# YuemingJin/STswinCL

Measured on AMD Instinct MI355X. Metric: input frames/s, TswinPlus fwd+bwd+Adam, 4-frame 512x512 clips, higher is better.
Workload: dtype bf16; 1 GPU; BASELINE.json configs[1]: TswinPlus(12) seg train step, 4 clips/GPU x T=4 frames x 3x512x512, swin res (64,64), OHEM-CE, Adam; T=4 because the reference asserts it (swin_512.py:313); clips_per_gpu=4, frames_per_clip=4, parallelism=dp1, graph_requested=True

## Files before the change

### include/stswin_hip.h

```cpp
#ifndef STSWIN_HIP_H
#define STSWIN_HIP_H
#ifdef __cplusplus
extern "C" {
#endif

#define STSWIN_GF_GELU 1
#define STSWIN_GF_RESID 2
#define STSWIN_GF_MUL_DGELU 4
#define STSWIN_GF_OUT_F32 8
#define STSWIN_GF_ACCUM 16
#define STSWIN_GF_RELU 32
#define STSWIN_GF_MUL_R 8192
#define STSWIN_GF_C2_DGELU 16384
#define STSWIN_GF_CS_PARTIAL 32768
#define STSWIN_GF_CS_SQ 65536
#define STSWIN_GF_TAPSKIP (1 << 29)
#define STSWIN_GF_BIG 128
#define STSWIN_GF_MID 512
#define STSWIN_GF_NOPIPE 1024
#define STSWIN_GF_HALF 2048
#define STSWIN_GF_M32PP (1u << 31)
#define STSWIN_GF_W4R (1 << 30)
#define STSWIN_GF_ROT 4096
#define STSWIN_GF_NOBIG 256
// ... 86 lines not shown
#define STSWIN_VAR_TN_RING_BSEG 23
#define STSWIN_VAR_TN_128x128 30
#define STSWIN_VAR_TN_128x128_W4 31
#define STSWIN_VAR_TN_ROWS 32
#define STSWIN_VAR_TN_SLABS_F32 0x1000
#define STSWIN_VAR_TN_SLABS_BF16 0x2000
#define STSWIN_VAR_TN_FUSED 0x8000
#define STSWIN_VAR_TN_TAPMINOR 0x4000
#define STSWIN_TN_OUT_TAPMINOR (1 << 25)
int stswin_gemm_nt_qkv_fp8(const void* A, long lda, const int* a_rows, const void* B, long ldb, void* out8, long ld8, float* scales,
                           long ld_scales, const float* bias, int M, int N, int Kseg, float scale, int scale_cols, int rows_per_problem,
                           int head_dim, void* stream);
int stswin_win_attn_fwd_f8(const void* qkv8, long ld8, const float* scales, long ld_scales, void* out, long ldo, const float* biasT,
                           const float* maskT, int nB_, int nW, int T_frames, int ws, int heads, int C, int bias_windows,
                           const int* bias_index, void* stream);
int stswin_win_attn_bwd_f8(const void* qkv8, long ld8, const float* scales, long ld_scales, const void* dout, long lddo, void* dqkv, long lddq,
                           const float* biasT, const float* maskT, float* dbiasT, float* dqkv_colsum, int nB_, int nW, int T_frames, int ws,
                           int heads, int C, float scale, int bias_windows, const int* bias_index, float* scratch, long scratch_floats,
                           void* stream);
int stswin_last_variant(int family);
int stswin_tuning_build(void);

int stswin_slab_fold(const float* ws, long slab_stride, long ws_batch_stride, int nslabs, int seg_len, int nseg, float* out0, float* out1,
                     float* out2, long out_batch_stride, int batch, int accumulate, void* stream);

int stswin_fold_defer(int on, void* stream);
int stswin_fold_flush(void* stream);

long stswin_colsum_scratch(int M, int N);
int stswin_colsum(int dtype, const void* y, long ldy, float* out, int M, int N, float* scratch, void* stream);

int stswin_layernorm_fwd(int dtype, const void* x, long ldx, const int* rows, int S, int Cseg, void* y, long ldy,
                         const float* gamma, const float* beta, float* mean, float* rstd, int M, float eps, void* stream);
int stswin_layernorm_bwd(int dtype, const void* dy, long lddy, const void* x, long ldx, const int* rows, int S, int Cseg,
                         const float* gamma, const float* mean, const float* rstd, void* dx, long lddx, float* dgamma,
                         float* dbeta, int M, int accumulate_dx,
                         float* dxsum ,
                         float* scratch ,
                         void* stream);
int stswin_layernorm_bwd_add(int dtype, const void* dy, long lddy, const void* x, long ldx, const int* rows, int S, int Cseg,
                             const float* gamma, const float* mean, const float* rstd, const void* add, long ldadd, void* dx, long lddx,
                             float* dgamma, float* dbeta, int M, float* dxsum, float* scratch, void* stream);
long stswin_layernorm_bwd_scratch(int M, int C);

int stswin_vec_gather(const float* v, const int* map, float* out, int n, float fill, void* stream);
int stswin_vec_gather_multi(int count, const float* const* v, const int* map, float* const* out, int n, const float* fill, void* stream);

int stswin_bias_expand(const float* table, const long* index, const float* mask, float* out, int N, int heads, int nW,
                       void* stream);
int stswin_bias_expand_multi(int count, const float* const* table, const long* const* index, const float* const* mask, float* const* out,
                             const int* N, const int* heads, const int* nW, void* stream);
int stswin_bias_scatter(const float* dbiasT, const int* order, const int* offs, float* dtable, int N, int heads, int table_rows, int nslabs,
                        void* stream);

int stswin_win_attn_fwd(int dtype, const void* qkv, long ld, void* out, long ldo, const float* biasT, const float* maskT,
                        int nB_, int nW, int T_frames, int ws, int heads, int C, int bias_windows,
                        const int* bias_index, void* stream);
int stswin_win_attn_qkv_fwd(const void* x, long ldx, long x_rows, const int* rmap, const void* w, long ldw, const float* bqkv, void* qkv_out,
                            long ldq, void* out, long ldo, const float* biasT, int nB_, int nW, int T_frames, int ws, int heads, int C,
                            float scale, int bias_windows, const int* bias_index, void* stream);
int stswin_win_attn_fwd_fp8(const void* qkv, long ld, void* out, long ldo, const float* biasT, const float* maskT, int nB_, int nW,
                            int T_frames, int ws, int heads, int C, int bias_windows, const int* bias_index, void* stream);
int stswin_win_attn_bwd(int dtype, const void* qkv, long ld, const void* dout, long lddo, void* dqkv, long lddq,
                        const float* biasT, const float* maskT, float* dbiasT,
                        float* dqkv_q_colsum ,
                        int nB_, int nW, int T_frames, int ws,
                        int heads, int C, float scale, int bias_windows, const int* bias_index,
                        float* scratch , long scratch_floats, void* stream);
long stswin_win_attn_bwd_scratch(int nB_, int ws, int heads, int C);

int stswin_colstats(int dtype, const void* x, long ldx, float* sum , float* sumsq , int M, int C, int groups, int unit_rows,
                    float* scratch , void* stream);
long stswin_colstats_scratch(int dtype, int M, int C, int groups, int unit_rows);
int stswin_cs_group_reduce(const float* table, int M, int N, int groups, int unit_rows, float* sum, float* sumsq, void* stream);

int stswin_bn_table_finalize(const float* table, int M, int N, int groups, int unit_rows, float* mean, float* rstd,
                             float* running_mean, float* running_var, float eps, float momentum, void* stream);
int stswin_bn_finalize(int dtype, const void* x, long ldx, const float* sum, const float* sumsq, float* mean, float* rstd,
                       float* running_mean, float* running_var, int M, int C, int groups, float eps, float momentum,
                       int unit_rows, void* stream);
int stswin_bn_apply(int dtype, const void* x, long ldx, const float* mean, const float* rstd, const float* gamma,
                    const float* beta, const void* resid, long ldr, void* y, long ldy, int M, int C, int groups, int relu,
                    int unit_rows, void* stream);
int stswin_bn_bwd(int dtype, const void* dy, long lddy, const void* x, long ldx,
                  const void* y ,
                  long ldy, const float* mean, const float* rstd, const float* gamma, const float* beta ,
                  float* s1, float* s2, void* dx, long lddx, void* dresid, long lddr,
                  int M, int C, int groups, int relu, int training,
                  int phase ,
                  long rows_total , int unit_rows,
                  float* group_sums ,
                  float* scratch ,
                  void* stream);
long stswin_bn_bwd_scratch(int dtype, int M, int C, int groups, int unit_rows);
int stswin_bn_relu_pool(int dtype, const void* x, long ldx, const float* mean, const float* rstd, const float* gamma, const float* beta,
                        void* out, long ldo, unsigned char* arg, int frames, int H, int W, int C, int groups, int unit_rows, void* stream);
int stswin_rows_broadcast(int dtype, const float* v, void* out, long ldo, int M, int C, int groups, float scale,
                          int accumulate, void* stream);
int stswin_bilinear(int dtype, const void* in, long ldi, void* out, long ldo, int frames, int h, int w, int H, int W, int C,
                    int backward, void* stream);
int stswin_logits_upsample(int dtype, const void* tokens, long ldt, void* nchw, int frames, int h, int w, int H, int W,
                           int nc, int backward, void* stream);

int stswin_ce_fwd(int dtype, const void* logits, const long* labels, float* loss, float* stats, int frames, long HW, int nc,
                  int ignore_index, float thresh, void* stream);
#define STSWIN_OHEM_WORK_BYTES (3 * 2048 * 12 + 48)
int stswin_ohem_select(const float* loss, long n, long n_min, float thresh, const float* stats, void* work, long work_bytes,
                       float* value, float* sel, void* stream);
int stswin_ce_bwd(int dtype, const void* logits, const long* labels, const float* loss, const float* sel,
                  const float* gscale, void* dlogits, int frames, long HW, int nc, int ignore_index, void* stream);

int stswin_contrast_fwd(int dtype, const void* Q, long ldq, const void* const* K5, long ldk, const int* lq,
                        const int* const* lk5, float* pos, float* all, int N, int HW, int C, void* stream);

int stswin_contrast_bank_fwd(int dtype, const void* Q, long ldq, const int* lq, int M, int C, int q_sets, int q_block,
                             const void* bank, long ldb, const int* lb, int maps, int seg, int bank_block, int groups,
                             const int* gmap , float inv_tau, float* pos, float* all,
                             float* rowmax, float* lse, float* workspace, long workspace_floats, void* stream);
int stswin_contrast_bank_fwd_unit(int dtype, const void* Q, long ldq, const int* lq, int M, int C, int q_sets, int q_block,
                             const void* bank, long ldb, const int* lb, int maps, int seg, int bank_block, int groups,
                             const int* gmap , float inv_tau, float* pos, float* all,
                             float* rowmax, float* lse, float* workspace, long workspace_floats, void* stream);
int stswin_contrast_class_sums(int dtype, const void* bank, long ldb, const int* lb, int maps, int seg, int bank_block, int C,
                               int ncls, float* ksum, float* scratch , void* stream);
long stswin_contrast_class_sums_scratch(int maps, int seg, int bank_block, int C, int ncls);
int stswin_contrast_bank_dq(const float* dpos, const float* dneg, const float* cnt, const int* lq, const float* ksum, float* dq,
                            long lddq, int M, int C, int q_sets, int q_block, int seg, int bank_block, int ncls, int groups, const int* gmap,
                            void* stream);

int stswin_rownorm_scatter(int dtype, const void* X, long ldx, void* Y, long ldy, float* inv, int R, int C, int views, int HW, int samples,
                           void* stream);
int stswin_rownorm_scatter_bwd(int dtype, const void* X, long ldx, const float* inv, const float* dY, long lddy, void* dX, long lddx, int R,
                               int C, int views, int HW, int samples, void* stream);
int stswin_labels_resize(const float* const* masks, int maps, int N, int Hs, int Ws, int h, int w, int* lb, void* stream);
int stswin_label_counts(const int* lq, const int* lb, int M, int maps, int seg, int q_sets, int q_block, int bank_block, int ncls, int groups,
                        const int* gmap, int* hist, float* cnt, void* stream);
int stswin_pair_loss(const float* pos, const float* all, const float* cnt, int M, int groups, int q_sets, int visible, float* loss,
                     void* stream);
int stswin_pair_loss_bwd(const float* pos, const float* all, const float* cnt, const float* dloss, int M, int groups, int q_sets, int visible,
                         float* dpos, float* dneg, void* stream);

int stswin_upsample_argmax(int dtype, const void* logits, unsigned char* labels, const long* gt, int* counts, int frames,
                           int nc, int h, int w, int H, int W, void* stream);
int stswin_upsample_argmax_cm(int dtype, const void* logits, unsigned char* labels, const long* gt, unsigned long long* cm, int ncm,
                              int align_corners, int frames, int nc, int h, int w, int H, int W, void* stream);

int stswin_frame_ingest(const unsigned char* in, unsigned char* tmp, float* out, int n, int Hs, int Ws, int H, int W,
                        const int* hbounds, const int* hcoef, int hksize, const int* vbounds, const int* vcoef, int vksize,
                        const float* lut, void* stream);
int stswin_frame_ingest_planes(const unsigned char* in, unsigned char* tmp, float* out, int n, int Hs, int Ws, int H, int W,
                               const int* hbounds, const int* hcoef, int hksize, const int* vbounds, const int* vcoef, int vksize,
                               const float* lut, void* stream);
int stswin_clip_assemble(int dtype, void* ring, const void* fresh, void* clips, const int* table, int B, int n_store, int slots,
                         int n_fresh, long frame_elems, void* stream);

int stswin_multi_tensor(int mode, int count, void* const* p, const void* const* g, void* const* m, void* const* v,
                        const int* n, float lr, float b1, float b2, float eps, float wd, float c1, float c2, void* stream);

int stswin_multi_tensor_lars(int count, void* const* p, const void* const* g, void* const* m, const int* n, float* norms,
                             long norms_floats, float lr, float momentum, float wd, float trust_coef, float eps, int first, int adaptive,
                             void* stream);

int stswin_optim_tick(int kind, int* counter, float* hyper, double a, double b, void* stream);
int stswin_multi_tensor_dev(int mode, int count, void* const* p, const void* const* g, void* const* m, void* const* v, const int* n,
                            const float* hyper, float b1, float b2, float eps, float wd, int first, void* stream);
int stswin_multi_tensor_lars_dev(int count, void* const* p, const void* const* g, void* const* m, const int* n, float* norms,
// ... 13 lines not shown
```

### stswincl_amd/csrc/headops.hip

```cpp
#include "common.h"
#include <cstdlib>

static int reduce_rows_per_chunk(int group_rows, int other_blocks, int nrl) {
  int rpc = 8 * nrl;
  while (rpc < 64 * nrl && (long)other_blocks * ((group_rows + 2 * rpc - 1) / (2 * rpc)) >= 1024) rpc *= 2;
  return rpc;
}
static int bn_bwd_rows(long rows_all_groups, int col_blocks, int nrl, int max_rows) {
  static const int tgt_red = getenv("STSWIN_BN_RED_WGS") ? atoi(getenv("STSWIN_BN_RED_WGS")) : 512;
  static const int tgt_dx = getenv("STSWIN_BN_DX_WGS") ? atoi(getenv("STSWIN_BN_DX_WGS")) : 2048;
  const int tgt = max_rows > 32 ? tgt_red : tgt_dx;
  int rows = 8;
  while (rows < max_rows && (long)col_blocks * (rows_all_groups / ((long)2 * rows * nrl)) >= tgt) rows *= 2;
  return rows;
}

DEVI long group_row0(int g, int ch, int rows_per_chunk, int group_rows, int unit, int G) {
  if (unit <= 0) return (long)g * group_rows;
  return ((long)((ch * rows_per_chunk) / unit) * (G - 1) + g) * unit;
}
DEVI long group_first_row(int g, int group_rows, int unit) { return unit > 0 ? (long)g * unit : (long)g * group_rows; }
static int fit_chunk(int rpc, int unit) {
  if (unit <= 0) return rpc;
  while (rpc > 1 && unit % rpc) rpc >>= 1;
// ... 473 lines not shown
    return;
  }
  float mx = -3.0e38f;
  for (int c = 0; c < nc; ++c) mx = fmaxf(mx, to_f32<TL>(b[(long)c * HW]));
  float s = 0.f;
  for (int c = 0; c < nc; ++c) s += expf(to_f32<TL>(b[(long)c * HW]) - mx);
  const float inv = 1.f / s;
  for (int c = 0; c < nc; ++c) {
    const float pr = expf(to_f32<TL>(b[(long)c * HW]) - mx) * inv;
    d[(long)c * HW] = from_f32<TL>(wgt * (pr - (c == lab ? 1.f : 0.f)));
  }
}

#define PACK_OF(dt) ((dt) == 0 ? 8 : 4)
#define DISPATCH_T(dt, CALL_BF16, CALL_F32) do { if ((dt) == 0) { CALL_BF16; } else { CALL_F32; } } while (0)

static int colstats_geometry(int dtype, int M, int C, int groups, int unit_rows, int* cpb_o, int* rpc_o, int* cpg_o) {
  if (C % PACK_OF(dtype) || groups <= 0 || M % groups) return -1401;
  if (unit_rows > 0 && M % ((long)groups * unit_rows)) return -1405;
  const int ppr = C / PACK_OF(dtype), cpb = pick_cpb(ppr);
  const int gr = M / groups, rpc = fit_chunk(reduce_rows_per_chunk(gr, groups * ((ppr + cpb - 1) / cpb), 256 / cpb), unit_rows);
  if (rpc <= 0) return -1405;
  *cpb_o = cpb; *rpc_o = rpc; *cpg_o = (gr + rpc - 1) / rpc;
  return 0;
}
extern "C" long stswin_colstats_scratch(int dtype, int M, int C, int groups, int unit_rows) {
  int cpb, rpc, cpg;
  const int rc = colstats_geometry(dtype, M, C, groups, unit_rows, &cpb, &rpc, &cpg);
  return rc ? rc : (long)groups * cpg * 2 * C;
}

extern "C" int stswin_colstats(int dtype, const void* x, long ldx, float* sum, float* sumsq, int M, int C, int groups,
                               int unit_rows, float* scratch, void* stream) {
  int cpb, rpc, cpg;
  const int rc = colstats_geometry(dtype, M, C, groups, unit_rows, &cpb, &rpc, &cpg);
  if (rc) return rc;
  if (ldx % PACK_OF(dtype)) return -1401;
  if (!scratch) return -1406;
  const int ppr = C / PACK_OF(dtype), gr = M / groups;
  dim3 grid((ppr + cpb - 1) / cpb, groups * cpg);
  hipStream_t st = (hipStream_t)stream;
  if (sumsq)
    DISPATCH_T(dtype, hipLaunchKernelGGL((colstats_kernel<bf16, true>), grid, dim3(256), 0, st, (const bf16*)x, ldx, scratch, C, gr, cpg, rpc, cpb, unit_rows),
               hipLaunchKernelGGL((colstats_kernel<float, true>), grid, dim3(256), 0, st, (const float*)x, ldx, scratch, C, gr, cpg, rpc, cpb, unit_rows));
  else
    DISPATCH_T(dtype, hipLaunchKernelGGL((colstats_kernel<bf16, false>), grid, dim3(256), 0, st, (const bf16*)x, ldx, scratch, C, gr, cpg, rpc, cpb, unit_rows),
               hipLaunchKernelGGL((colstats_kernel<float, false>), grid, dim3(256), 0, st, (const float*)x, ldx, scratch, C, gr, cpg, rpc, cpb, unit_rows));
  const int rf = stswin_fold_launch(scratch, 2L * C, (long)cpg * 2 * C, cpg, C, sumsq ? 2 : 1, sum, sumsq, nullptr, C, groups, 1, st);
  if (rf) return rf;
  STSWIN_CHECK_LAUNCH();
  return 0;
}

extern "C" int stswin_bn_finalize(int dtype, const void* x, long ldx, const float* sum, const float* sumsq, float* mean,
                                  float* rstd, float* running_mean, float* running_var, int M, int C, int groups, float eps,
                                  float momentum, int unit_rows, void* stream) {
  if (groups <= 0 || M % groups) return -1401;
  hipStream_t st = (hipStream_t)stream;
  dim3 grid((C + 255) / 256);
  DISPATCH_T(dtype, hipLaunchKernelGGL(bn_finalize_kernel<bf16>, grid, dim3(256), 0, st, (const bf16*)x, ldx, sum, sumsq, mean, rstd, running_mean, running_var, C, groups, M / groups, eps, momentum, unit_rows),
             hipLaunchKernelGGL(bn_finalize_kernel<float>, grid, dim3(256), 0, st, (const float*)x, ldx, sum, sumsq, mean, rstd, running_mean, running_var, C, groups, M / groups, eps, momentum, unit_rows));
  STSWIN_CHECK_LAUNCH();
  return 0;
}

extern "C" int stswin_bn_apply(int dtype, const void* x, long ldx, const float* mean, const float* rstd, const float* gamma,
                               const float* beta, const void* resid, long ldr, void* y, long ldy, int M, int C, int groups,
                               int relu, int unit_rows, void* stream) {
  const int pk = PACK_OF(dtype);
  if (C % pk || ldx % pk || ldy % pk || (resid && ldr % pk) || groups <= 0 || M % groups) return -1402;
  const int ppr = C / pk, cpb = pick_cpb(ppr);
  if (unit_rows > 0 && M % ((long)groups * unit_rows)) return -1405;
  const int gr = M / groups, rpc = fit_chunk(8 * (256 / cpb), unit_rows);
  if (rpc <= 0) return -1405;
  const int cpg = (gr + rpc - 1) / rpc;
  dim3 grid((ppr + cpb - 1) / cpb, groups * cpg);
  hipStream_t st = (hipStream_t)stream;
  DISPATCH_T(dtype, hipLaunchKernelGGL(bn_apply_kernel<bf16>, grid, dim3(256), 0, st, (const bf16*)x, ldx, mean, rstd, gamma, beta, (const bf16*)resid, ldr, (bf16*)y, ldy, C, gr, cpg, rpc, relu, cpb, unit_rows),
             hipLaunchKernelGGL(bn_apply_kernel<float>, grid, dim3(256), 0, st, (const float*)x, ldx, mean, rstd, gamma, beta, (const float*)resid, ldr, (float*)y, ldy, C, gr, cpg, rpc, relu, cpb, unit_rows));
  STSWIN_CHECK_LAUNCH();
  return 0;
}

static int bn_bwd_geometry(int dtype, int M, int C, int groups, int unit_rows, int* cpb_o, int* rpc_o, int* rpc2_o) {
  const int pk = PACK_OF(dtype);
  if (C % pk || groups <= 0 || M % groups) return -1403;
  if (unit_rows > 0 && M % ((long)groups * unit_rows)) return -1405;
  const int ppr = C / pk, cpb = pick_cpb(ppr), xb = (ppr + cpb - 1) / cpb, nrl = 256 / cpb;
  const int rpc = fit_chunk(bn_bwd_rows(M, xb, nrl, 64) * nrl, unit_rows);
  const int rpc2 = fit_chunk(bn_bwd_rows(M, xb, nrl, 32) * nrl, unit_rows);
  if (rpc <= 0 || rpc2 <= 0) return -1405;
  *cpb_o = cpb; *rpc_o = rpc; *rpc2_o = rpc2;
  return 0;
}
extern "C" long stswin_bn_bwd_scratch(int dtype, int M, int C, int groups, int unit_rows) {
  int cpb, rpc, rpc2;
  const int rc = bn_bwd_geometry(dtype, M, C, groups, unit_rows, &cpb, &rpc, &rpc2);
  return rc ? rc : (long)groups * ((M / groups + rpc - 1) / rpc) * 2 * C;
}

extern "C" int stswin_bn_bwd(int dtype, const void* dy, long lddy, const void* x, long ldx, const void* y, long ldy,
                             const float* mean, const float* rstd, const float* gamma, const float* beta, float* s1, float* s2,
                             void* dx, long lddx, void* dresid, long lddr, int M, int C, int groups, int relu, int training,
                             int phase, long rows_total, int unit_rows, float* gsum, float* scratch, void* stream) {
  const int pk = PACK_OF(dtype);
  int cpb, rpc, rpc2;
  const int rc = bn_bwd_geometry(dtype, M, C, groups, unit_rows, &cpb, &rpc, &rpc2);
  if (rc) return rc;
  if (ldx % pk || lddy % pk || lddx % pk || (relu && y && ldy % pk)) return -1403;
  if (relu && !y && !beta) return -1404;
  if (phase != 2 && !scratch) return -1406;
  const int ppr = C / pk, gr = M / groups;
  const int cpg = (gr + rpc - 1) / rpc;
  dim3 g1((ppr + cpb - 1) / cpb, groups * cpg);
  const int cpg2 = (gr + rpc2 - 1) / rpc2;
  dim3 g2((ppr + cpb - 1) / cpb, groups * cpg2);
  hipStream_t st = (hipStream_t)stream;
  const float inv_n = 1.0f / (float)(rows_total > 0 ? rows_total : gr);
  if (phase != 2) {
    DISPATCH_T(dtype, hipLaunchKernelGGL(bn_bwd_reduce_kernel<bf16>, g1, dim3(256), 0, st, (const bf16*)dy, lddy, (const bf16*)x, ldx, (const bf16*)y, ldy, mean, rstd, scratch, C, gr, cpg, rpc, relu, cpb, gamma, beta, unit_rows),
               hipLaunchKernelGGL(bn_bwd_reduce_kernel<float>, g1, dim3(256), 0, st, (const float*)dy, lddy, (const float*)x, ldx, (const float*)y, ldy, mean, rstd, scratch, C, gr, cpg, rpc, relu, cpb, gamma, beta, unit_rows));
    const int rf = stswin_fold_launch(scratch, 2L * C, (long)cpg * 2 * C, cpg, C, 2, s1, s2, nullptr, C, groups, 1, st);
    if (rf) return rf;
  }
  if (phase != 1)
  DISPATCH_T(dtype, hipLaunchKernelGGL(bn_bwd_dx_kernel<bf16>, g2, dim3(256), 0, st, (const bf16*)dy, lddy, (const bf16*)x, ldx, (const bf16*)y, ldy, mean, rstd, gamma, s1, s2, (bf16*)dx, lddx, (bf16*)dresid, lddr, C, gr, cpg2, rpc2, relu, training, cpb, inv_n, beta, unit_rows, gsum),
             hipLaunchKernelGGL(bn_bwd_dx_kernel<float>, g2, dim3(256), 0, st, (const float*)dy, lddy, (const float*)x, ldx, (const float*)y, ldy, mean, rstd, gamma, s1, s2, (float*)dx, lddx, (float*)dresid, lddr, C, gr, cpg2, rpc2, relu, training, cpb, inv_n, beta, unit_rows, gsum));
  STSWIN_CHECK_LAUNCH();
  return 0;
}

template <typename T>
__global__ __launch_bounds__(256) void bn_relu_pool_kernel(const T* x, long ldx, const float* mean, const float* rstd, const float* gamma,
                                                            const float* beta, T* out, long ldo, unsigned char* arg, int frames, int H,
                                                            int W, int Hp, int Wp, int C, int G, int group_rows, int unit) {
  constexpr int PACK = TT<T>::PACK;
  const int ppr = C / PACK, Hb = (Hp + 1) >> 1, Wb = (Wp + 1) >> 1;
  const long idx = (long)blockIdx.x * 256 + threadIdx.x;
  if (idx >= (long)frames * Hb * Wb * ppr) return;
  const int c = (int)(idx % ppr) * PACK;
  const long pb = idx / ppr;
  const int xb = (int)(pb % Wb), yb = (int)((pb / Wb) % Hb);
  const long f = pb / ((long)Wb * Hb);
  const long row0 = f * H * W;
  const int g = unit > 0 ? (int)((row0 / unit) % G) : (int)(row0 / group_rows);
  float sc[8], sh[8], best[4][8];
  unsigned char ba[4][8];
#pragma unroll
  for (int e = 0; e < PACK; ++e) {
    const float rs = rstd[(long)g * C + c + e] * gamma[c + e];
    sc[e] = rs;
    sh[e] = beta[c + e] - mean[(long)g * C + c + e] * rs;
#pragma unroll
    for (int o = 0; o < 4; ++o) { best[o][e] = -3.0e38f; ba[o][e] = 255; }
  }
  const int y0 = 4 * yb - 1, x0 = 4 * xb - 1;
#pragma unroll
  for (int iy = 0; iy < 5; ++iy) {
    const int yy = y0 + iy;
    if (yy < 0 || yy >= H) continue;
#pragma unroll
    for (int ix = 0; ix < 5; ++ix) {
      const int xx = x0 + ix;
      if (xx < 0 || xx >= W) continue;
      Vec16<T> v, z;
      v.v = *(const decltype(v.v)*)(x + (row0 + (long)yy * W + xx) * ldx + c);
// ... 497 lines not shown
```

### stswincl_amd/headops.py

```python
from __future__ import annotations

import os
import weakref
from typing import List, Optional, Sequence, Tuple

import torch
import torch.nn.functional as F

from . import hip
from .ops import compute_dtype, _f32

KGRAN = 64


_INDEX_MAPS = {}
_TORCH_PADVEC = os.environ.get("STSWIN_TORCH_PADVEC") == "1"
_BN_KEEP_Y = os.environ.get("STSWIN_BN_KEEP_Y") == "1"


class Layout:

    def __init__(self, segs: Sequence[Tuple[int, int, int]], width: int):
        self.segs, self.width = list(segs), width
        self.logical = sum(s[1] for s in self.segs)
# ... 362 lines not shown
def combine_bn_stats(mean_r: torch.Tensor, m2_r: torch.Tensor, n_r: torch.Tensor):
    n = n_r.sum()
    w = (n_r / n).view(-1, 1, 1)
    mean = (mean_r * w).sum(0)
    m2 = (m2_r + n_r.view(-1, 1, 1) * (mean_r - mean) ** 2).sum(0)
    return mean, m2 / n, n


def refuse_replica(module) -> None:
    if getattr(module, "_is_replica", False):
        raise hip.StswinHipError(
            "stswincl_amd modules do not run as nn.DataParallel replicas (several GPUs driven by threads of one process). Use one "
            "process per GPU instead: `python -m torch.distributed.run --nproc-per-node N train.py` with "
            "torch.nn.parallel.DistributedDataParallel or stswincl_amd.dp.GradBucketReducer (see INTEGRATION.md, 'Data parallel'); "
            "nn.DataParallel(model, device_ids=[torch.cuda.current_device()]) - a single device - is fine.")


COLLECTIVES: dict = {}


def _sync_world(bn) -> int:
    import torch.distributed as dist
    if isinstance(bn, torch.nn.SyncBatchNorm) and dist.is_available() and dist.is_initialized():
        return dist.get_world_size()
    return 1


def rowmajor(t: torch.Tensor, dt) -> torch.Tensor:
    t = t.detach()
    if t.dtype != dt:
        t = t.to(dt)
    if (t.dim() == 2 and t.stride(1) == 1 and (t.stride(0) * t.element_size()) % 16 == 0 and t.data_ptr() % 16 == 0
            and t.stride(0) >= t.shape[1]):
        return t
    return t.contiguous()


class ConcatColsFn(torch.autograd.Function):

    @staticmethod
    def forward(ctx, buf, widths, *parts):
        off = 0
        for w_, p_ in zip(widths, parts):
            assert p_.data_ptr() == buf.data_ptr() + off * buf.element_size() and p_.shape[1] == w_ and p_.stride(0) == buf.stride(0), \
                "ConcatColsFn: a part does not live in its column slice of the buffer"
            off += w_
        assert off == buf.shape[1]
        ctx.widths = widths
        return buf.view_as(buf)

    @staticmethod
    def backward(ctx, g):
        outs, off = [], 0
        for w_ in ctx.widths:
            outs.append(g[:, off:off + w_])
            off += w_
        return (None, None, *outs)


def concat_buffer(rows: int, widths, dt, device):
    buf = torch.empty(rows, sum(widths), dtype=dt, device=device)
    views, off = [], 0
    for w_ in widths:
        views.append(buf[:, off:off + w_])
        off += w_
    return buf, views


class BNTokFn(torch.autograd.Function):

    @staticmethod
    def forward(ctx, x, gamma, beta, running_mean, running_var, training, relu, resid, groups, lay, eps, momentum, world=1,
                unit=0, stats=None, link=None, out=None):
        ctx.link = link
        dt = compute_dtype(x)
        X = x.detach().to(dt)
        M, Cp = X.shape
        assert Cp == lay.width
        fused_pad = training and world == 1 and not lay.is_identity
        if fused_pad:
            gp, bp, rm_p, rv_p = lay.pad_vecs([gamma, beta, running_mean, running_var], [0.0, 0.0, 0.0, 1.0])
        else:
            gp, bp = lay.pad_vec(gamma), lay.pad_vec(beta)
        rows_total = 0
        if training and world > 1:
            import torch.distributed as dist
            n_loc = M // groups
            s, ss = hip.colstats(X, groups=groups, unit=unit)
            pivot = (X.view(-1, unit, Cp)[:groups, 0, :] if unit > 0 else X.view(groups, n_loc, Cp)[:, 0, :]).float()
            mean_l = pivot + s / n_loc
            m2_l = ss - s * s / n_loc
            pack = torch.stack([mean_l, m2_l, torch.full_like(mean_l, float(n_loc))])
            allp = torch.empty(world * 3, *pack.shape[1:], dtype=pack.dtype, device=pack.device)
            dist.all_gather_into_tensor(allp, pack)
            COLLECTIVES["syncbn_all_gather"] = COLLECTIVES.get("syncbn_all_gather", 0) + 1
            allp = allp.view(world, 3, *pack.shape[1:])
            n_r = allp[:, 2, 0, 0]
            mean, var, n_tot = combine_bn_stats(allp[:, 0], allp[:, 1], n_r)
            rstd = torch.rsqrt(var + eps)
            unbias = n_tot / (n_tot - 1).clamp(min=1)
            ctx.sum_scale = float(n_loc) / n_tot
            rm, rv = lay.pad_vec(running_mean), lay.pad_vec(running_var, 1.0)
            for g in range(groups):
                rm = (1 - momentum) * rm + momentum * mean[g]
                rv = (1 - momentum) * rv + momentum * var[g] * unbias
            running_mean.copy_(lay.unpad_vec(rm))
            running_var.copy_(lay.unpad_vec(rv))
            mean, rstd = mean.contiguous(), rstd.contiguous()
        elif training:
            raw = stats is not None and groups <= 32 and ((unit % 256 == 0) if unit > 0 else ((M // groups) % 256 == 0))

            def finalize(rm, rv):
                if raw:
                    return hip.bn_table_finalize(stats, M, rm, rv, groups, eps, momentum, unit=unit)
                s, ss = hip.colstats(X, groups=groups, unit=unit)
                return hip.bn_finalize(X, s, ss, rm, rv, groups, eps, momentum, unit=unit)

            if lay.is_identity:
                mean, rstd = finalize(running_mean, running_var)
            else:
                mean, rstd = finalize(rm_p, rv_p)
                lay.unpad_vecs([rm_p, rv_p], into=[running_mean, running_var])
        else:
            mean = lay.pad_vec(running_mean).view(1, Cp).expand(groups, Cp).contiguous()
            rstd = torch.rsqrt(lay.pad_vec(running_var, 1.0) + eps).view(1, Cp).expand(groups, Cp).contiguous()
        if out is not None:
            assert out.shape == (M, Cp) and out.dtype == dt and out.stride(1) == 1
            y = out.view_as(out)
        else:
            y = torch.empty(M, Cp, dtype=dt, device=x.device)
        R = resid.detach().to(dt) if resid is not None else None
        hip.bn_apply(X, mean, rstd, gp, bp, y, resid=R, groups=groups, relu=relu, unit=unit)
        ctx.cfg = (training, relu, groups, lay, dt, x.dtype, resid is not None, world, rows_total)
        ctx.unit = unit
        keep_y = relu and (resid is not None or _BN_KEEP_Y)
        ctx.save_for_backward(X, y if keep_y else None, mean, rstd, gp, bp if relu else None)
        return y

    @staticmethod
    def backward(ctx, dy):
        X, y, mean, rstd, gp, bp = ctx.saved_tensors
        training, relu, groups, lay, dt, in_dtype, has_res, world, rows_total = ctx.cfg
        g = rowmajor(dy, dt)
        dx = torch.empty_like(X)
        dres = torch.empty_like(X) if has_res else None
        if training and world > 1:
            import torch.distributed as dist
            s1, s2 = hip.bn_bwd(g, X, y if relu else None, mean, rstd, gp, dx, dres, groups, relu, training, phase=1, beta=bp,
                                unit=ctx.unit)
            loc1, loc2 = s1.clone(), s2.clone()
            both = torch.stack([s1, s2])
            dist.all_reduce(both)
            COLLECTIVES["syncbn_all_reduce"] = COLLECTIVES.get("syncbn_all_reduce", 0) + 1
            both = both * ctx.sum_scale
            hip.bn_bwd(g, X, y if relu else None, mean, rstd, gp, dx, dres, groups, relu, training, phase=2,
                       sums=(both[0].contiguous(), both[1].contiguous()), rows_total=0, beta=bp, unit=ctx.unit)
            s1, s2 = loc1, loc2
        else:
            gs = torch.empty(2, X.shape[1], dtype=torch.float32, device=X.device) if groups > 1 else None
            s1, s2 = hip.bn_bwd(g, X, y if relu else None, mean, rstd, gp, dx, dres, groups, relu, training, beta=bp, unit=ctx.unit,
                                group_sums=gs)
            if gs is not None:
                s1, s2, groups = gs[0:1], gs[1:2], 1
        if groups > 1:
            if s1._base is not None and s2._base is s1._base and s2.storage_offset() == s1.storage_offset() + s1.numel():
                both = torch.as_strided(s1, (2, groups, s1.shape[-1]), (groups * s1.shape[-1], s1.shape[-1], 1)).sum(1)
                s1, s2 = both[0:1], both[1:2]
            else:
                s1, s2 = s1.sum(0, keepdim=True), s2.sum(0, keepdim=True)
        if lay.is_identity:
            dgamma, dbeta = s2[0], s1[0]
        else:
            dgamma, dbeta = lay.unpad_vecs([s2[0].contiguous(), s1[0].contiguous()])
        dres = dres.to(in_dtype) if has_res else None
        if dres is not None and ctx.link is not None:
            ctx.link.put(dres)
            dres = None
        return (dx.to(in_dtype), dgamma, dbeta, None, None, None, None, dres, None, None, None, None, None, None, None, None, None)


class BNTokGroupFn(torch.autograd.Function):

    @staticmethod
    def forward(ctx, n, *args):
        import torch.distributed as dist
        cfgs, tens = args[:n], args[n:]
        world = dist.get_world_size()
        st, packs = [], []
        for i in range(n):
            relu, groups, lay, eps, momentum, unit, out = cfgs[i]
            x, gamma, beta, rmean, rvar = tens[5 * i:5 * i + 5]
            dt = compute_dtype(x)
            X = x.detach().to(dt)
            M, Cp = X.shape
            assert Cp == lay.width
            n_loc = M // groups
            s, ss = hip.colstats(X, groups=groups, unit=unit)
            pivot = (X.view(-1, unit, Cp)[:groups, 0, :] if unit > 0 else X.view(groups, n_loc, Cp)[:, 0, :]).float()
            mean_l = pivot + s / n_loc
            m2_l = ss - s * s / n_loc
            packs.append(torch.stack([mean_l, m2_l, torch.full_like(mean_l, float(n_loc))]).reshape(3, groups * Cp))
            st.append((X, dt, M, Cp, n_loc, x.dtype))
        pack = torch.cat(packs, dim=1).contiguous()
        allp = torch.empty(world * 3, pack.shape[1], dtype=pack.dtype, device=pack.device)
        dist.all_gather_into_tensor(allp, pack)
        COLLECTIVES["syncbn_all_gather"] = COLLECTIVES.get("syncbn_all_gather", 0) + 1
        allp = allp.view(world, 3, -1)
        outs, saved, meta, off = [], [], [], 0
        for i in range(n):
            relu, groups, lay, eps, momentum, unit, out = cfgs[i]
            x, gamma, beta, rmean, rvar = tens[5 * i:5 * i + 5]
            X, dt, M, Cp, n_loc, in_dtype = st[i]
            blk = allp[:, :, off:off + groups * Cp].reshape(world, 3, groups, Cp)
            off += groups * Cp
            n_r = blk[:, 2, 0, 0]
# ... 385 lines not shown
```

### stswincl_amd/hip.py

```python
from __future__ import annotations

import ctypes
import functools
import os
import re
from typing import Optional

import torch

_ROOT = os.path.dirname(os.path.dirname(os.path.abspath(__file__)))
LIB_PATH = os.environ.get("STSWIN_HIP_LIB") or os.path.join(_ROOT, "stswincl_amd", "lib", "libstswin_hip.so")
HEADER_PATH = os.path.join(_ROOT, "include", "stswin_hip.h")
_lib: Optional[ctypes.CDLL] = None

_c_int, _c_float, _c_void_p = ctypes.c_int, ctypes.c_float, ctypes.c_void_p


class StswinHipError(RuntimeError):
    pass


_C_TYPES = {"int": ctypes.c_int, "long": ctypes.c_long, "float": ctypes.c_float, "double": ctypes.c_double}


# ... 862 lines not shown
                                        _p(dqkv), _ld(dqkv), _p(biasT), _p(maskT), _p(dbiasT), _p(colsum_out), nB_, nW, T, ws, heads, C,
                                        scale, _bias_windows(biasT, maskT, nW, bias_index), _p(bias_index), _p(sc),
                                        sc.numel(), _stream())
    _check(rc, "win_attn_bwd_f8")
    return dqkv


def win_attn_qkv_fwd(x, rmap, w, bqkv, biasT, *, nB_, nW, T, ws, heads, C, scale, bias_index=None, want_qkv=True, debug_ts=None):
    rows = nB_ * T * ws * ws
    if x.dtype != torch.bfloat16 or w.dtype != torch.bfloat16:
        raise StswinHipError("win_attn_qkv_fwd is a bf16 kernel")
    out = torch.empty(rows, C, dtype=x.dtype, device=x.device)
    qkv = torch.empty(rows, 3 * C, dtype=x.dtype, device=x.device) if want_qkv else None
    if debug_ts is not None:
        rc = load().stswin_win_attn_qkv_fwd(_p(x), _ld(x), x.shape[0], _p(rmap), _p(w), _ld(w), _p(bqkv), _p(debug_ts), 0,
                                            _p(out), _ld(out), _p(biasT), nB_, nW, T, ws, heads, C, scale,
                                            _bias_windows(biasT, None, nW, bias_index) | _ATTN_DEBUG_STAMPS, _p(bias_index), _stream())
        _check(rc, "win_attn_qkv_fwd")
        return out, None
    name = "attn_qkv_fwd_bf16"
    with _Span(name, 2.0 * rows * 3 * C * C + 4.0 * nB_ * heads * (T * ws * ws) ** 2 * (C // heads)):
        rc = load().stswin_win_attn_qkv_fwd(_p(x), _ld(x), x.shape[0], _p(rmap), _p(w), _ld(w), _p(bqkv), _p(qkv),
                                            _ld(qkv) if qkv is not None else 0, _p(out), _ld(out), _p(biasT), nB_, nW, T,
                                            ws, heads, C, scale, _bias_windows(biasT, None, nW, bias_index), _p(bias_index),
                                            _stream())
    _check(rc, "win_attn_qkv_fwd")
    return out, qkv


def win_attn_qkv_fwd_ok(x: torch.Tensor) -> bool:
    return x.shape[0] * _ld(x) * 2 <= 0xFFFF0000


def win_attn_bwd(qkv, dout, biasT, maskT, dbiasT, *, nB_, nW, T, ws, heads, C, scale, colsum_out=None, debug_ts=False,
                 bias_index=None):
    dqkv = torch.empty_like(qkv)
    lib = load()
    need = lib.stswin_win_attn_bwd_scratch(nB_, ws, heads, C)
    if need < 0:
        raise StswinHipError(f"win_attn_bwd: bad geometry ({need})")
    sc = scratch(qkv.device, need)
    rc = load().stswin_win_attn_bwd(_dt(qkv), _p(qkv), _ld(qkv), _p(dout), _ld(dout), _p(dqkv),
                                    _ld(dqkv), _p(biasT), _p(maskT), _p(dbiasT), _p(colsum_out), nB_, nW, T, ws, heads, C,
                                    scale, _bias_windows(biasT, maskT, nW, bias_index) | (_ATTN_DEBUG_STAMPS if debug_ts else 0),
                                    _p(bias_index), _p(sc), sc.numel(), _stream())
    _check(rc, "win_attn_bwd")
    return dqkv


def colstats(x, groups=1, squares=True, M=None, unit=0):
    M = x.shape[0] if M is None else M
    C = x.shape[1]
    both = zeros(2 if squares else 1, groups, C, device=x.device)
    s = both[0]
    ss = both[1] if squares else None
    lib = load()
    need = lib.stswin_colstats_scratch(_dt(x), M, C, groups, unit)
    if need < 0:
        raise StswinHipError(f"colstats: bad geometry ({need})")
    _check(lib.stswin_colstats(_dt(x), _p(x), _ld(x), _p(s), _p(ss), M, C, groups, unit, _p(scratch(x.device, need)), _stream()),
           "colstats")
    return s, ss


def bn_finalize(x, s, ss, running_mean, running_var, groups=1, eps=1e-5, momentum=0.1, M=None, unit=0, raw=False):
    M = x.shape[0] if M is None else M
    C = x.shape[1]
    mean = torch.empty(groups, C, dtype=torch.float32, device=x.device)
    rstd = torch.empty(groups, C, dtype=torch.float32, device=x.device)
    _check(load().stswin_bn_finalize(_dt(x), _p(None if raw else x), _ld(x), _p(s), _p(ss), _p(mean), _p(rstd), _p(running_mean),
                                     _p(running_var), M, C, groups, eps, momentum, unit, _stream()),
           "bn_finalize")
    return mean, rstd


def bn_apply(x, mean, rstd, gamma, beta, out, resid=None, groups=1, relu=True, M=None, unit=0):
    M = x.shape[0] if M is None else M
    _check(load().stswin_bn_apply(_dt(x), _p(x), _ld(x), _p(mean), _p(rstd), _p(gamma), _p(beta), _p(resid),
                                  _ld(resid) if resid is not None else 0, _p(out), _ld(out), M,
                                  x.shape[1], groups, 1 if relu else 0, unit, _stream()), "bn_apply")
    return out


def bn_bwd(dy, x, y, mean, rstd, gamma, dx, dresid=None, groups=1, relu=True, training=True, M=None, phase=0, sums=None,
           rows_total=0, beta=None, unit=0, group_sums=None):
    M = x.shape[0] if M is None else M
    C = x.shape[1]
    if sums is None:
        both = zeros(2, groups, C, device=x.device)
        s1, s2 = both[0], both[1]
    else:
        s1, s2 = sums
    lib = load()
    need = lib.stswin_bn_bwd_scratch(_dt(x), M, C, groups, unit) if phase != 2 else 0
    if need < 0:
        raise StswinHipError(f"bn_bwd: bad geometry ({need})")
    _check(lib.stswin_bn_bwd(_dt(x), _p(dy), _ld(dy), _p(x), _ld(x), _p(y),
                                _ld(y) if y is not None else 0, _p(mean), _p(rstd), _p(gamma), _p(beta), _p(s1), _p(s2),
                                _p(dx), _ld(dx), _p(dresid), _ld(dresid) if dresid is not None else 0, M, C,
                                groups, 1 if relu else 0, 1 if training else 0, phase, rows_total, unit, _p(group_sums),
                                _p(scratch(x.device, need) if phase != 2 else None), _stream()), "bn_bwd")
    return s1, s2


def bn_relu_pool(x, mean, rstd, gamma, beta, frames, H, W, groups=1, unit=0):
    C = x.shape[1]
    Hp, Wp = (H - 1) // 2 + 1, (W - 1) // 2 + 1
    out = torch.empty(frames * Hp * Wp, C, dtype=x.dtype, device=x.device)
    arg = torch.empty(frames * Hp * Wp, C, dtype=torch.uint8, device=x.device)
    _check(load().stswin_bn_relu_pool(_dt(x), _p(x), _ld(x), _p(mean), _p(rstd), _p(gamma), _p(beta), _p(out), _ld(out),
                                      _p(arg), frames, H, W, C, groups, unit, _stream()), "bn_relu_pool")
    return out, arg


def rows_broadcast(v, out, groups, scale=1.0, accumulate=False, M=None):
    M = out.shape[0] if M is None else M
    _check(load().stswin_rows_broadcast(_dt(out), _p(v), _p(out), _ld(out), M, v.shape[1], groups,
                                        scale, 1 if accumulate else 0, _stream()), "rows_broadcast")
    return out


def bilinear(src, dst, frames, h, w, H, W, backward=False):
    C = dst.shape[1]
    _check(load().stswin_bilinear(_dt(src), _p(src), _ld(src), _p(dst), _ld(dst), frames, h, w, H, W, C,
                                  1 if backward else 0, _stream()), "bilinear")
    return dst


def logits_upsample(tokens, nchw, frames, h, w, H, W, nc, backward=False):
    _check(load().stswin_logits_upsample(_dt(tokens), _p(tokens), _ld(tokens), _p(nchw), frames, h, w, H, W, nc,
                                         1 if backward else 0, _stream()), "logits_upsample")


def ce_fwd(logits, labels, ignore_index, thresh):
    F_, nc = logits.shape[:2]
    HW = logits[0, 0].numel()
    loss = torch.empty(F_ * HW, dtype=torch.float32, device=logits.device)
    stats = zeros(4, device=logits.device)
    _check(load().stswin_ce_fwd(_dt(logits), _p(logits), _p(labels), _p(loss), _p(stats), F_, HW, nc, ignore_index,
                                thresh, _stream()), "ce_fwd")
    return loss, stats


def ohem_select(loss, stats, n_min: int, thresh: float):
    work = torch.empty(OHEM_WORK_BYTES // 4, dtype=torch.int32, device=loss.device)
    value = torch.empty((), dtype=torch.float32, device=loss.device)
    sel = torch.empty(4, dtype=torch.float32, device=loss.device)
    _check(load().stswin_ohem_select(_p(loss), loss.numel(), n_min, thresh, _p(stats), _p(work),
                                     OHEM_WORK_BYTES, _p(value), _p(sel), _stream()), "ohem_select")
    return value, sel


def ce_bwd(logits, labels, loss, sel, gscale, ignore_index):
    F_, nc = logits.shape[:2]
    HW = logits[0, 0].numel()
    d = torch.empty_like(logits)
    _check(load().stswin_ce_bwd(_dt(logits), _p(logits), _p(labels), _p(loss), _p(sel), _p(gscale), _p(d), F_, HW,
                                nc, ignore_index, _stream()), "ce_bwd")
    return d


def contrast_fwd(q, keys, lq, lks, N, HW):
    C = q.shape[1]
    assert len(keys) == 5 and len(lks) == 5 and all(k.dtype == q.dtype and _ld(k) == _ld(keys[0]) for k in keys)
    pos = torch.empty(N, HW, 5, dtype=torch.float32, device=q.device)
    tot = torch.empty(N, HW, 5, dtype=torch.float32, device=q.device)
# ... 310 lines not shown
```

Before: 618.8 frames/s.

## Fuse BN stats, finalize and apply into one kernel for small-row inputs

Adds a single-kernel batch-norm forward path for layers with at most 1024 rows. Each block computes pivot-shifted column sums over all rows, finalizes mean, rstd and running stats, then applies scale, shift, residual and ReLU. This replaces the separate colstats, finalize and apply launches. The aim is to cut launch overhead and an extra read of x on the small, low-resolution BN layers, at the cost of a grid with few blocks that only parallelizes over channels.

```diff
diff --git a/include/stswin_hip.h b/include/stswin_hip.h
--- a/include/stswin_hip.h
+++ b/include/stswin_hip.h
@@ -192,6 +192,11 @@
 int stswin_bn_apply(int dtype, const void* x, long ldx, const float* mean, const float* rstd, const float* gamma,
                     const float* beta, const void* resid, long ldr, void* y, long ldy, int M, int C, int groups, int relu,
                     int unit_rows, void* stream);
+int stswin_bn_small_eligible(int dtype, int M, int C, int groups, int unit_rows);
+int stswin_bn_small_max_rows(void);
+int stswin_bn_fwd_small(int dtype, const void* x, long ldx, const float* gamma, const float* beta, const void* resid, long ldr,
+                        void* y, long ldy, float* mean, float* rstd, float* running_mean, float* running_var, int M, int C,
+                        int groups, int relu, float eps, float momentum, int unit_rows, void* stream);
 int stswin_bn_bwd(int dtype, const void* dy, long lddy, const void* x, long ldx,
                   const void* y ,
                   long ldy, const float* mean, const float* rstd, const float* gamma, const float* beta ,
diff --git a/stswincl_amd/csrc/headops.hip b/stswincl_amd/csrc/headops.hip
--- a/stswincl_amd/csrc/headops.hip
+++ b/stswincl_amd/csrc/headops.hip
@@ -579,6 +579,170 @@
   return 0;
 }
 
+#define SMALL_THREADS 512
+#define SMALL_MAX_ROWS_DEFAULT 1024
+#define SMALL_W_DEFAULT 8
+DEVI long group_phys_row(int g, int r, int group_rows, int unit, int G) {
+  if (unit <= 0) return (long)g * group_rows + r;
+  return ((long)(r / unit) * G + g) * unit + r % unit;
+}
+template <typename T, int W>
+__global__ __launch_bounds__(SMALL_THREADS) void bn_fwd_small_kernel(
+    const T* x, long ldx, const float* gamma, const float* beta, const T* resid, long ldr, T* y, long ldy, float* mean, float* rstd,
+    float* running_mean, float* running_var, int C, int G, int group_rows, int unit, int relu, float eps, float momentum,
+    int nrl, int rpc, int cpg, int QL) {
+  constexpr int PACK = TT<T>::PACK, SL = SMALL_THREADS / W, CH = W * 8;
+  __shared__ __attribute__((aligned(16))) float part[SL * W * 16];
+  __shared__ float acc[2][64 * CH];
+  const int t = threadIdx.x, cp = t % W, sl = t / W;
+  const int c = (blockIdx.x * W + cp) * PACK;
+  const int NS = cpg * nrl;
+  const int fj = t % CH, fq0 = t / CH;
+  const int fcc = (blockIdx.x * W + (fj >> 3)) * PACK + (fj & 7);
+  const bool fvalid = (fj & 7) < PACK && fcc < C;
+  float rm = 0.f, rv = 0.f;
+  if (t < CH && fvalid && running_mean) { rm = running_mean[fcc]; rv = running_var[fcc]; }
+  for (int g = 0; g < G; ++g) {
+    for (int i = t; i < QL * CH; i += W * SL) { acc[0][i] = 0.f; acc[1][i] = 0.f; }
+    float pv[8] = {0, 0, 0, 0, 0, 0, 0, 0};
+    if (c < C) {
+      Vec16<T> p0;
+      p0.v = *(const decltype(p0.v)*)(x + group_first_row(g, group_rows, unit) * ldx + c);
+#pragma unroll
+      for (int e = 0; e < PACK; ++e) pv[e] = p0.get(e);
+    }
+    for (int s0 = 0; s0 < NS; s0 += SL) {
+      float a1[8] = {0, 0, 0, 0, 0, 0, 0, 0}, a2[8] = {0, 0, 0, 0, 0, 0, 0, 0};
+      const int s = s0 + sl;
+      if (c < C && s < NS) {
+        const int ch = s / nrl, rl = s % nrl;
+        const int r_end = min(group_rows, (ch + 1) * rpc);
+        for (int r = ch * rpc + rl; r < r_end; r += 8 * nrl) {
+          Vec16<T> in[8];
+#pragma unroll
+          for (int u = 0; u < 8; ++u)
+            if (r + u * nrl < r_end) in[u].v = *(const decltype(in[u].v)*)(x + group_phys_row(g, r + u * nrl, group_rows, unit, G) * ldx + c);
+#pragma unroll
+          for (int u = 0; u < 8; ++u)
+            if (r + u * nrl < r_end) {
+#pragma unroll
+              for (int e = 0; e < PACK; ++e) {
+                const float d = in[u].get(e) - pv[e];
+                a1[e] += d;
+                a2[e] += d * d;
+              }
+            }
+        }
+      }
+#pragma unroll
+      for (int e = 0; e < 8; ++e) { part[(sl * W + cp) * 16 + e] = a1[e]; part[(sl * W + cp) * 16 + 8 + e] = a2[e]; }
+      __syncthreads();
+      if (fvalid) {
+        const int p_lo = s0 / nrl, p_hi = min(cpg, (s0 + SL) / nrl);
+        for (int q = fq0; q < QL; q += (W * SL) / CH) {
+          int p = p_lo + ((q - p_lo) % QL + QL) % QL;
+          for (; p < p_hi; p += QL) {
+            float s1 = 0.f, s2 = 0.f;
+            const float* pp = part + ((p - p_lo) * nrl * W + (fj >> 3)) * 16 + (fj & 7);
+            for (int k = 0; k < nrl; ++k) { s1 += pp[k * W * 16]; s2 += pp[k * W * 16 + 8]; }
+            acc[0][q * CH + fj] += s1;
+            acc[1][q * CH + fj] += s2;
+          }
+        }
+      }
+      __syncthreads();
+    }
+    if (t < CH && fvalid) {
+      float sum = acc[0][fj], sumsq = acc[1][fj];
+      for (int k = 1; k < QL; ++k) { sum += acc[0][k * CH + fj]; sumsq += acc[1][k * CH + fj]; }
+      sum = 0.f + sum;
+      sumsq = 0.f + sumsq;
+      const float pivot = to_f32<T>(x[group_first_row(g, group_rows, unit) * ldx + fcc]);
+      const float ms = sum / group_rows;
+      const float var = fmaxf(sumsq / group_rows - ms * ms, 0.f);
+      const float mu = pivot + ms, rsd = rsqrtf(var + eps);
+      mean[(long)g * C + fcc] = mu;
+      rstd[(long)g * C + fcc] = rsd;
+      rm = (1.f - momentum) * rm + momentum * (pivot + ms);
+      rv = (1.f - momentum) * rv + momentum * var * ((float)group_rows / (float)max(group_rows - 1, 1));
+      const float rs = rsd * gamma[fcc];
+      part[(fj >> 3) * PACK + (fj & 7)] = rs;
+      part[CH + (fj >> 3) * PACK + (fj & 7)] = beta[fcc] - mu * rs;
+    }
+    __syncthreads();
+    if (c < C) {
+      float sc[8], sh[8];
+#pragma unroll
+      for (int e = 0; e < PACK; e += 4) {
+        *(f32x4*)(sc + e) = *(const f32x4*)&part[cp * PACK + e];
+        *(f32x4*)(sh + e) = *(const f32x4*)&part[CH + cp * PACK + e];
+      }
+      for (int r = sl; r < group_rows; r += 8 * SL) {
+        Vec16<T> in[8], rs[8];
+#pragma unroll
+        for (int u = 0; u < 8; ++u)
+          if (r + u * SL < group_rows) {
+            const long row = group_phys_row(g, r + u * SL, group_rows, unit, G);
+            in[u].v = *(const decltype(in[u].v)*)(x + row * ldx + c);
+            if (resid) rs[u].v = *(const decltype(rs[u].v)*)(resid + row * ldr + c);
+          }
+#pragma unroll
+        for (int u = 0; u < 8; ++u)
+          if (r + u * SL < group_rows) {
+            const long row = group_phys_row(g, r + u * SL, group_rows, unit, G);
+            Vec16<T> o;
+#pragma unroll
+            for (int e = 0; e < PACK; ++e) {
+              float v = in[u].get(e) * sc[e] + sh[e];
+              if (resid) v += rs[u].get(e);
+              if (relu) v = fmaxf(v, 0.f);
+              o.set(e, v);
+            }
+            *(decltype(o.v)*)(y + row * ldy + c) = o.v;
+          }
+      }
+    }
+    __syncthreads();
+  }
+  if (t < CH && fvalid && running_mean) { running_mean[fcc] = rm; running_var[fcc] = rv; }
+}
+
+extern "C" int stswin_bn_small_max_rows(void) {
+  static const int max_rows = getenv("STSWIN_BN_SMALL_ROWS") ? atoi(getenv("STSWIN_BN_SMALL_ROWS")) : SMALL_MAX_ROWS_DEFAULT;
+  return max_rows;
+}
+extern "C" int stswin_bn_small_eligible(int dtype, int M, int C, int groups, int unit_rows) {
+  const int max_rows = stswin_bn_small_max_rows();
+  int cpb, rpc, cpg;
+  if (dtype != 0 && dtype != 1) return 0;
+  if (M <= 0 || M > max_rows) return 0;
+  if (colstats_geometry(dtype, M, C, groups, unit_rows, &cpb, &rpc, &cpg)) return 0;
+  if (256 / cpb > SMALL_THREADS / 8) return 0;
+  return 1;
+}
+
+extern "C" int stswin_bn_fwd_small(int dtype, const void* x, long ldx, const float* gamma, const float* beta, const void* resid, long ldr,
+                                   void* y, long ldy, float* mean, float* rstd, float* running_mean, float* running_var, int M, int C,
+                                   int groups, int relu, float eps, float momentum, int unit_rows, void* stream) {
+  const int pk = PACK_OF(dtype);
+  int cpb, rpc, cpg;
+  const int rc = colstats_geometry(dtype, M, C, groups, unit_rows, &cpb, &rpc, &cpg);
+  if (rc) return rc;
+  if (ldx % pk || ldy % pk || (resid && ldr % pk)) return -1402;
+  if (!stswin_bn_small_eligible(dtype, M, C, groups, unit_rows)) return -1407;
+  if ((running_mean == nullptr) != (running_var == nullptr)) return -1402;
+  const int ppr = C / pk, QL = cpg >= 96 ? 64 : 16;
+  static const int w_env = getenv("STSWIN_BN_SMALL_W") ? atoi(getenv("STSWIN_BN_SMALL_W")) : 0;
+  const int Wd = w_env == 1 || w_env == 2 || w_env == 4 || w_env == 8 ? w_env : SMALL_W_DEFAULT;
+  dim3 grid((ppr + Wd - 1) / Wd);
+  hipStream_t st = (hipStream_t)stream;
+#define BN_SMALL_LAUNCH(T, WW) hipLaunchKernelGGL((bn_fwd_small_kernel<T, WW>), grid, dim3(SMALL_THREADS), 0, st, (const T*)x, ldx, gamma, beta, (const T*)resid, ldr, (T*)y, ldy, mean, rstd, running_mean, running_var, C, groups, M / groups, unit_rows, relu, eps, momentum, 256 / cpb, rpc, cpg, QL)
+#define BN_SMALL_W(T) do { if (Wd == 1) BN_SMALL_LAUNCH(T, 1); else if (Wd == 2) BN_SMALL_LAUNCH(T, 2); else if (Wd == 4) BN_SMALL_LAUNCH(T, 4); else BN_SMALL_LAUNCH(T, 8); } while (0)
+  DISPATCH_T(dtype, BN_SMALL_W(bf16), BN_SMALL_W(float));
+  STSWIN_CHECK_LAUNCH();
+  return 0;
+}
+
 static int bn_bwd_geometry(int dtype, int M, int C, int groups, int unit_rows, int* cpb_o, int* rpc_o, int* rpc2_o) {
   const int pk = PACK_OF(dtype);
   if (C % pk || groups <= 0 || M % groups) return -1403;
diff --git a/stswincl_amd/headops.py b/stswincl_amd/headops.py
--- a/stswincl_amd/headops.py
+++ b/stswincl_amd/headops.py
@@ -468,7 +468,14 @@
             gp, bp, rm_p, rv_p = lay.pad_vecs([gamma, beta, running_mean, running_var], [0.0, 0.0, 0.0, 1.0])
         else:
             gp, bp = lay.pad_vec(gamma), lay.pad_vec(beta)
+        if out is not None:
+            assert out.shape == (M, Cp) and out.dtype == dt and out.stride(1) == 1
+            y = out.view_as(out)
+        else:
+            y = torch.empty(M, Cp, dtype=dt, device=x.device)
+        R = resid.detach().to(dt) if resid is not None else None
         rows_total = 0
+        applied = False
         if training and world > 1:
             import torch.distributed as dist
             n_loc = M // groups
@@ -495,10 +502,14 @@
             mean, rstd = mean.contiguous(), rstd.contiguous()
         elif training:
             raw = stats is not None and groups <= 32 and ((unit % 256 == 0) if unit > 0 else ((M // groups) % 256 == 0))
+            applied = not raw and hip.bn_small_eligible(X, groups=groups, unit=unit)
 
             def finalize(rm, rv):
                 if raw:
                     return hip.bn_table_finalize(stats, M, rm, rv, groups, eps, momentum, unit=unit)
+                if applied:
+                    return hip.bn_fwd_small(X, gp, bp, rm, rv, y, resid=R, groups=groups, relu=relu, eps=eps, momentum=momentum,
+                                            unit=unit)
                 s, ss = hip.colstats(X, groups=groups, unit=unit)
                 return hip.bn_finalize(X, s, ss, rm, rv, groups, eps, momentum, unit=unit)
 
@@ -510,13 +521,8 @@
         else:
             mean = lay.pad_vec(running_mean).view(1, Cp).expand(groups, Cp).contiguous()
             rstd = torch.rsqrt(lay.pad_vec(running_var, 1.0) + eps).view(1, Cp).expand(groups, Cp).contiguous()
-        if out is not None:
-            assert out.shape == (M, Cp) and out.dtype == dt and out.stride(1) == 1
-            y = out.view_as(out)
-        else:
-            y = torch.empty(M, Cp, dtype=dt, device=x.device)
-        R = resid.detach().to(dt) if resid is not None else None
-        hip.bn_apply(X, mean, rstd, gp, bp, y, resid=R, groups=groups, relu=relu, unit=unit)
+        if not applied:
+            hip.bn_apply(X, mean, rstd, gp, bp, y, resid=R, groups=groups, relu=relu, unit=unit)
         ctx.cfg = (training, relu, groups, lay, dt, x.dtype, resid is not None, world, rows_total)
         ctx.unit = unit
         keep_y = relu and (resid is not None or _BN_KEEP_Y)
diff --git a/stswincl_amd/hip.py b/stswincl_amd/hip.py
--- a/stswincl_amd/hip.py
+++ b/stswincl_amd/hip.py
@@ -968,6 +968,23 @@
     return out
 
 
+def bn_small_eligible(x, groups=1, M=None, unit=0) -> bool:
+    M = x.shape[0] if M is None else M
+    return bool(load().stswin_bn_small_eligible(_dt(x), M, x.shape[1], groups, unit))
+
+
+def bn_fwd_small(x, gamma, beta, running_mean, running_var, out, resid=None, groups=1, relu=True, eps=1e-5, momentum=0.1, M=None,
+                 unit=0):
+    M = x.shape[0] if M is None else M
+    C = x.shape[1]
+    mean = torch.empty(groups, C, dtype=torch.float32, device=x.device)
+    rstd = torch.empty(groups, C, dtype=torch.float32, device=x.device)
+    _check(load().stswin_bn_fwd_small(_dt(x), _p(x), _ld(x), _p(gamma), _p(beta), _p(resid), _ld(resid) if resid is not None else 0,
+                                      _p(out), _ld(out), _p(mean), _p(rstd), _p(running_mean), _p(running_var), M, C, groups,
+                                      1 if relu else 0, eps, momentum, unit, _stream()), "bn_fwd_small")
+    return mean, rstd
+
+
 def bn_bwd(dy, x, y, mean, rstd, gamma, dx, dresid=None, groups=1, relu=True, training=True, M=None, phase=0, sums=None,
            rows_total=0, beta=None, unit=0, group_sums=None):
     M = x.shape[0] if M is None else M
```

After: 620.0 frames/s, median of 4. No clear change (+0.2%).
